# yzhang511/multi_modal_foundation_model

Measured on AMD Instinct MI355X. Metric: pretrain samples/sec (T=100 bins/modality, d_model=256, 5+5 layers, spike+behaviour masked pretraining step), higher is better.
Workload: dtype bf16; 1 GPU; BASELINE.json configs[1]: 1 session, ap(668 neurons)+behaviour(2), d_model=256, heads=8, mlp=512, 5 enc + 5 dec layers, T=100 (L=200 tokens), dropout 0.4/0.2, AdamW+OneCycleLR, mixed objectives; per_gpu_batch=1024, global_batch=1024, seq_len=200, parallelism=dp1

## Files before the change

### include/mmfm.h

```cpp
#ifndef MMFM_H
#define MMFM_H
#include <stdint.h>
#ifdef __cplusplus
extern "C" {
#endif

#define MMFM_VERSION 401
#define MMFM_F32 0
#define MMFM_BF16 1
#define MMFM_NULL_BIAS 1
#define MMFM_EMBED_OPTS 1
#define MMFM_MLP_DX_ONLY 1
#define MMFM_MLP_GELU 0
#define MMFM_MLP_RELU 1
#define MMFM_MLP_SIGMOID 2
#define MMFM_MLP_GELU_TANH 3

typedef void* mmfm_stream;

typedef struct {
    const void* state;
    uint32_t site;
    float p;
} mmfm_dropout;
// ... 253 lines not shown
int mmfm_optim_ranges_table(const mmfm_optim_range* ranges, int n_ranges, int64_t n, int hyper_rows, void* table_host, int64_t table_bytes);
int64_t mmfm_optim_ranges_workspace(int64_t n_chunks, int n_ranges);
int mmfm_grad_sumsq_ranges(const float* g, int64_t n, const mmfm_optim_range* ranges, int n_ranges, const void* table, int64_t n_chunks,
                           float coef_in, float max_norm, int skip_nonfinite, void* workspace, int64_t workspace_bytes,
                           mmfm_stream stream);
int mmfm_adamw_step_ranges(float* p, const float* g, float* m, float* v, void* p_bf16, int64_t n, const mmfm_optim_range* ranges,
                           int n_ranges, const void* table, int64_t n_chunks, const float* hyper, int hyper_rows,
                           const mmfm_optim_record* record, int skip_nonfinite, mmfm_stream stream);

#define MMFM_GRAD_ACCUM 1
#define MMFM_GRAD_STASH 0
#define MMFM_GRAD_ADD 1
int mmfm_grad_accumulate(float* g, float* stash, int64_t n, int64_t start, int64_t end, int mode, mmfm_stream stream);

#define MMFM_SESSION_LINEAR 1
typedef struct {
    int dtype;
    int B, T, P, N_max, S;
    int ld_pad;
    int ld_p;
    const int32_t* sid;
    const int32_t* n;
    const int64_t* w_off;
    const int64_t* b_off;
    const void* w; int64_t w_elems;
    const float* bias; int64_t b_elems;
} mmfm_session_desc;
int mmfm_session_reduce(const mmfm_session_desc* d, const void* x_pad, void* y, mmfm_stream stream);
int mmfm_session_expand(const mmfm_session_desc* d, const void* f, void* y_pad, mmfm_stream stream);
int mmfm_session_dw_chunks(int B, int S, int chunk);
int64_t mmfm_session_runs_ints(int B, int S, int chunk);
int64_t mmfm_session_dw_workspace(int B, int P, int N_max, int S, int chunk);
int mmfm_session_dw(const mmfm_session_desc* d, const void* a_pad, const void* q, const int32_t* runs, int chunk, float* dw, float* db,
                    int bias_from_pad, void* workspace, int64_t workspace_bytes, mmfm_stream stream);

#define MMFM_SPAN_PACK 1
#define MMFM_SPAN_CHUNK 4096
#define MMFM_SPAN_MAX 65536
int mmfm_span_gather(const float* G, float* stage, const int64_t* table, int n_spans, mmfm_stream stream);
int mmfm_span_scatter(const float* stage, float* G, const int64_t* table, int n_spans, mmfm_stream stream);

int mmfm_r2_series(const float* gt, const int64_t* gt_strides, const float* pred, const int64_t* pred_strides,
                   int G, int S, int C, float* out, mmfm_stream stream);
int64_t mmfm_bits_per_spike_workspace(int64_t R, int N);
int mmfm_bits_per_spike(const float* rates, const float* spikes, int64_t R, int N, float* out,
                        void* workspace, int64_t workspace_bytes, mmfm_stream stream);
int64_t mmfm_bits_per_spike_neurons_workspace(int64_t R, int N);
int mmfm_bits_per_spike_neurons(const float* rates, const float* spikes, int64_t R, int N, float* out,
                                void* workspace, int64_t workspace_bytes, mmfm_stream stream);


typedef struct {
    const float* W;
    const float* gamma;
    const float* beta;
    const float* bias;
    void* Wp;
    void* WpT;
    float* bp;
    int N, K;
    int tile0;
    int scalar_gain;
    void* WpP;
    void* WpTP;
} mmfm_prep_entry;
int mmfm_prep_weights(const mmfm_prep_entry* entries, int n_entries, int total_tiles, mmfm_stream stream);

typedef struct {
    int64_t R;
    int K, N;
    const void* x; int ldx;
    const void* w; int ldw;
    const float* bias;
    int ln; float eps;
    void* xhat; float* rstd;
    const void* residual; int ldr;
    void* y; int ldy;
    int stream_out;
    int rotate;
    int ln_bwd;
    const void* bwd_xhat; const float* bwd_rstd;
} mmfm_rowgemm_desc;
int mmfm_rowgemm(const mmfm_rowgemm_desc* d, mmfm_stream stream);

#define MMFM_ROWGEMM_MAX_GROUPS 8
typedef struct {
    int64_t R;
    int K, N;
    int groups;
    const void* x[MMFM_ROWGEMM_MAX_GROUPS]; int ldx;
    const void* w[MMFM_ROWGEMM_MAX_GROUPS]; int ldw;
    const float* bias[MMFM_ROWGEMM_MAX_GROUPS];
    void* y[MMFM_ROWGEMM_MAX_GROUPS]; int ldy;
    int ln; float eps;
    void* xhat; float* rstd;
    const void* residual; int ldr;
    int stream_out, rotate;
    int ln_bwd;
    const void* bwd_xhat; const float* bwd_rstd;
} mmfm_rowgemm_groups_desc;
int mmfm_rowgemm_groups(const mmfm_rowgemm_groups_desc* d, mmfm_stream stream);

typedef struct {
    int64_t R;
    const void* x; int ldx;
    float eps;
    const void* w_up; const float* b_up;
    const void* w_down; const float* b_down;
    mmfm_dropout drop;
    void* y; int ldy;
    void* xhat; float* rstd;
    const void* dy; int lddy;
    const void* w_down_t;
    const void* w_up_t;
    void* t1; void* g; void* du;
    void* dx; int lddx;
    int rotate;
    int scalenorm;
    int act;
    float act_beta;
} mmfm_mlp_desc;
int mmfm_mlp_fwd(const mmfm_mlp_desc* d, mmfm_stream stream);
int mmfm_mlp_bwd(const mmfm_mlp_desc* d, mmfm_stream stream);

int64_t mmfm_ln_linear_grad_workspace(int K);
int mmfm_ln_linear_grad(const float* Gdb, const float* W, const float* gamma, const float* beta, int N, int K,
                        float* dW, float* dbias, float* dgamma, float* dbeta, int accumulate_ln,
                        void* workspace, int64_t workspace_bytes, mmfm_stream stream);
int mmfm_sn_linear_grad(const float* Gdb, const float* W, const float* g, int N, int K, float* dW, float* dbias, float* dg,
                        int accumulate, void* workspace, int64_t workspace_bytes, mmfm_stream stream);

int mmfm_mt19937_jump(uint32_t* state624, int32_t* consumed, uint64_t n);
int mmfm_mt19937_jump_reset(void);

#define MMFM_MT_DEVICE 1
#define MMFM_MT_MAX_STREAMS 1024
#define MMFM_MT_TABLES 64
int mmfm_mt_plan(uint64_t n, int streams, int32_t* out_streams, int64_t* out_blocks);
int64_t mmfm_mt_workspace(uint64_t n, int streams);
int mmfm_mt_uniform(const uint32_t* state624, int32_t consumed, uint64_t skip, uint64_t n, float* out, int streams,
                    void* workspace, int64_t workspace_bytes, mmfm_stream stream);
int mmfm_mt_bernoulli(const uint32_t* state624, int32_t consumed, uint64_t skip, uint64_t n, float p, uint8_t* out, int streams,
                      void* workspace, int64_t workspace_bytes, mmfm_stream stream);
int mmfm_mt_corrupt(const uint32_t* state624, int32_t consumed, int B, int T, int N, const float* src, const uint8_t* cm,
                    int64_t sb, int64_t st, int64_t sn, float zero_ratio, float random_ratio, float* dst, int streams,
                    void* workspace, int64_t workspace_bytes, mmfm_stream stream);

#ifdef __cplusplus
}
#endif
#endif
```

### multi_modal_foundation_model_amd/_lib.py

```python
from __future__ import annotations

import ctypes as C
import os
import re

import torch

_HERE = os.path.dirname(os.path.abspath(__file__))
LIB_PATH = os.environ.get("MMFM_LIB") or os.path.join(_HERE, "libmmfm_hip.so")
HEADER_PATH = os.path.join(os.path.dirname(_HERE), "include", "mmfm.h")

F32, BF16 = 0, 1
ATTN_DIAG, ATTN_CAUSAL, ATTN_SEP = 1, 2, 4
ATTN_FAMILY_KEEPBIT_DH32, ATTN_FAMILY_KEEPBIT_LONG, ATTN_FAMILY_BF16, ATTN_FAMILY_BF16_TILED, ATTN_FAMILY_F32, ATTN_FAMILY_F32_TILED = range(1, 7)
ATTN_FAMILY_MASK, ATTN_FAMILY_BWD_SINGLE = 0xf, 0x10
ATTN_KEEPBIT_FAMILIES = (ATTN_FAMILY_KEEPBIT_DH32, ATTN_FAMILY_KEEPBIT_LONG)
GEMM_FAMILY_F32, GEMM_FAMILY_TILE128, GEMM_FAMILY_BIG256, GEMM_FAMILY_DW128, GEMM_FAMILY_DW256 = range(1, 6)
ACT_NONE, ACT_GELU, ACT_SOFTSIGN, ACT_GELU_GRAD, ACT_SOFTSIGN_GRAD, ACT_SOFTSIGN_GRAD_OUT = 0, 1, 2, 3, 4, 5
ACT_RELU, ACT_RELU_GRAD, ACT_SIGMOID, ACT_SIGMOID_GRAD, ACT_GELU_TANH, ACT_GELU_TANH_GRAD = 6, 7, 8, 9, 10, 11
(ACT_EMB_IDENTITY, ACT_EMB_IDENTITY_GRAD, ACT_EMB_RELU, ACT_EMB_RELU_GRAD, ACT_EMB_GELU, ACT_EMB_GELU_GRAD, ACT_EMB_SILU, ACT_EMB_SILU_GRAD,
 ACT_EMB_QUICK_GELU, ACT_EMB_QUICK_GELU_GRAD, ACT_EMB_GELU_TANH, ACT_EMB_GELU_TANH_GRAD, ACT_EMB_TANH, ACT_EMB_TANH_GRAD) = range(12, 26)
MLP_GELU, MLP_RELU, MLP_SIGMOID, MLP_GELU_TANH = 0, 1, 2, 3
LOSS_POISSON_LOG, LOSS_MSE, LOSS_POISSON_RATE, LOSS_L1, LOSS_SMOOTH_L1, LOSS_HUBER, LOSS_BCE_LOGITS = range(7)
LOSS_FULL = 1
# ... 119 lines not shown
    "mmfm_last_error": (C.c_char_p, []),
    "mmfm_device_check": (C.c_int, [_i]),
    "mmfm_rng_seed": (C.c_int, [_vp, C.c_uint64, _vp]),
    "mmfm_rng_advance": (C.c_int, [_vp, _vp]),
    "mmfm_gemm": (C.c_int, [C.POINTER(GemmDesc), _vp]),
    "mmfm_gemm_pair": (C.c_int, [_vp, _vp, _vp]),
    "mmfm_gemm_live": (C.c_int, [C.POINTER(GemmDesc), C.POINTER(LiveRows), _vp]),
    "mmfm_gemm_family": (C.c_int, [C.POINTER(GemmDesc), C.POINTER(LiveRows)]),
    "mmfm_gemm_pair_fused": (C.c_int, [C.POINTER(GemmDesc), C.POINTER(GemmDesc)]),
    "mmfm_live_bins": (C.c_int, [_vp, _i, _i, _vp, _vp]),
    "mmfm_gather_live_rows": (C.c_int, [_vp, _vp, _i, _i, _i64, _vp, _vp]),
    "mmfm_gemm_dw_tiles": (C.c_int, [_i, _i, _i]),
    "mmfm_reduce_slabs": (C.c_int, [_vp, _vp, _i64, _i, _i64, _i, _vp]),
    "mmfm_reduce_slabs_multi": (C.c_int, [_vp, _i, _i, _vp]),
    "mmfm_colsum_workspace": (C.c_int64, [_i64, _i]),
    "mmfm_colsum": (C.c_int, [_i, _vp, _i64, _i, _i, _vp, _i, _vp, _i64, _vp]),
    "mmfm_layernorm_fwd": (C.c_int, [_i, _vp, _vp, _vp, _vp, _vp, _vp, _i64, _i, _f, _i, _i, _vp]),
    "mmfm_layernorm_bwd_workspace": (C.c_int64, [_i64, _i]),
    "mmfm_layernorm_bwd": (C.c_int, [_i, _vp, _vp, _vp, _vp, _vp, _vp, _vp, _vp, _vp, _i, _i64, _i, _i, _i, _vp, _i64, _vp]),
    "mmfm_scalenorm_fwd": (C.c_int, [_i, _vp, _vp, _vp, _vp, _i64, _i, _f, _vp]),
    "mmfm_scalenorm_bwd_workspace": (C.c_int64, [_i64, _i]),
    "mmfm_scalenorm_bwd": (C.c_int, [_i, _vp, _vp, _vp, _vp, _vp, _vp, _vp, _i, _i64, _i, _vp, _i64, _vp]),
    "mmfm_attn_fwd": (C.c_int, [C.POINTER(AttnDesc), _vp]),
    "mmfm_attn_bwd": (C.c_int, [C.POINTER(AttnDesc), _vp]),
    "mmfm_attn_keepbits_bytes": (C.c_int64, [_i, _i, _i, _i]),
    "mmfm_attn_keep_prob": (C.c_float, [_f]),
    "mmfm_attn_family": (C.c_int, [C.POINTER(AttnDesc), _i]),
    "mmfm_attn_win_fwd": (C.c_int, [C.POINTER(AttnDesc), C.POINTER(AttnWindow), _vp]),
    "mmfm_attn_win_bwd": (C.c_int, [C.POINTER(AttnDesc), C.POINTER(AttnWindow), _vp]),
    "mmfm_attn_win_family": (C.c_int, [C.POINTER(AttnDesc), C.POINTER(AttnWindow), _i]),
    "mmfm_attn_pos_prep": (C.c_int, [_i, _i, C.POINTER(C.c_int32), C.POINTER(_vp), _vp, _vp]),
    "mmfm_mask_prep": (C.c_int, [_i, _i, _i, C.POINTER(_vp), C.POINTER(_i64), _vp, C.POINTER(_i64), _vp, _vp, _vp, _vp, _vp, _vp]),
    "mmfm_collate_csr": (C.c_int, [_i, _i, _i, _f, _vp, _vp, _vp, _vp, _vp, _vp, _vp, _vp, _vp, _vp, _vp]),
    "mmfm_stitch_fwd": (C.c_int, [_i, _vp, _vp, _vp, _vp, _vp, _vp, _vp, _i, _i, _i, _i, _i, _i, _vp]),
    "mmfm_stitch_fwd_live": (C.c_int, [_i, _vp, _vp, _vp, _vp, _vp, _vp, _vp, _vp, _i, _i, _i, _i, _i, _i, _vp]),
    "mmfm_stitch_bwd_live": (C.c_int, [_i, _vp, _vp, _vp, _vp, _vp, Dropout, _vp, _vp, _vp, _i, _i, _i, _i, _i, _i, _i, _i, _vp, _i64, _vp]),
    "mmfm_stitch_bwd_workspace": (C.c_int64, [_i, _i, _i, _i, _i, _i]),
    "mmfm_stitch_bwd": (C.c_int, [_i, _vp, _vp, _vp, _vp, Dropout, _vp, _vp, _vp, _i, _i, _i, _i, _i, _i, _i, _i, _vp, _i64, _vp]),
    "mmfm_mask_prep_seg": (C.c_int, [_i, _i, C.POINTER(C.c_int32), C.POINTER(_vp), C.POINTER(_i64), C.POINTER(_vp), C.POINTER(_i64), _vp, _vp, _vp, _vp,
                                     _vp, _vp]),
    "mmfm_stitch_fwd_seg": (C.c_int, [_i, _vp, _vp, _vp, _vp, _vp, _vp, _vp, _i, _i, _i, _i, _i, _i, _vp]),
    "mmfm_stitch_bwd_seg_workspace": (C.c_int64, [_i, _i, _i, _i, _i, _i, _i]),
    "mmfm_stitch_bwd_seg": (C.c_int, [_i, _vp, _vp, _vp, _vp, Dropout, _vp, _vp, _vp, _i, _i, _i, _i, _i, _i, _i, _i, _vp, _i64, _vp]),
    "mmfm_layernorm_fwd_seg": (C.c_int, [_i, _vp, _vp, _vp, _vp, _vp, _vp, _i64, _i, _f, _i, C.POINTER(C.c_int32), _vp]),
    "mmfm_layernorm_bwd_seg": (C.c_int, [_i, _vp, _vp, _vp, _vp, _vp, _vp, _vp, _vp, _vp, _i, _i64, _i, _i, C.POINTER(C.c_int32), _vp, _i64, _vp]),
    "mmfm_masked_loss_workspace": (C.c_int64, [_i64, _i]),
    "mmfm_masked_loss_fwd": (C.c_int, [_i, _i, _vp, _vp, _vp, _i, _i, _i64, _i, _vp, _vp, _i64, _vp]),
    "mmfm_masked_loss_kind_fwd": (C.c_int, [_i, _i, _f, _i, _vp, _vp, _vp, _i, _i, _i64, _i, _vp, _vp, _i64, _vp]),
    "mmfm_loss_finalize": (C.c_int, [_vp, _vp, _i, _vp, _vp, _vp]),
    "mmfm_masked_loss_bwd": (C.c_int, [_i, _i, _vp, _vp, _vp, _i, _i, _i64, _i, _vp, _vp, _vp, _vp]),
    "mmfm_masked_loss_kind_bwd": (C.c_int, [_i, _i, _f, _i, _vp, _vp, _vp, _i, _i, _i64, _i, _vp, _vp, _vp, _vp]),
    "mmfm_masked_loss_elem_workspace": (C.c_int64, [_i64, _i]),
    "mmfm_masked_loss_elem_fwd": (C.c_int, [_i, _i, _f, _i, _vp, _vp, _vp, _i64, _i64, _i64, _i, _i, _i, _vp, _vp, _vp, _i64, _vp]),
    "mmfm_masked_loss_elem_bwd": (C.c_int, [_i, _i, _f, _i, _vp, _vp, _vp, _i64, _i64, _i64, _i, _i, _i, _vp, _vp, _vp, _vp]),
    "mmfm_stage_masked": (C.c_int, [_i, _vp, _vp, _i64, _i64, _i64, _i, _i, _i, _vp, _i, _vp]),
    "mmfm_masked_loss_chan_workspace": (C.c_int64, [_i64, _i]),
    "mmfm_masked_loss_chan_fwd": (C.c_int, [_i, _i, _f, _i, _vp, _vp, _vp, _i, _i, _i64, _i, _vp, _i, _vp, _vp, _vp, _i64, _vp]),
    "mmfm_masked_loss_chan_bwd": (C.c_int, [_i, _i, _f, _i, _vp, _vp, _vp, _i, _i, _i64, _i, _vp, _i, _vp, _vp, _vp, _vp]),
    "mmfm_softmax_ce_workspace": (C.c_int64, [_i64, _i]),
    "mmfm_softmax_ce_fwd": (C.c_int, [_i, _vp, _vp, _vp, _f, _vp, _i, _i, _i64, _i, _vp, _vp, _vp, _i64, _vp]),
    "mmfm_softmax_ce_bwd": (C.c_int, [_i, _vp, _vp, _vp, _f, _vp, _i, _i, _i64, _i, _vp, _vp, _vp, _vp, _vp]),
    "mmfm_argmax_confusion": (C.c_int, [_i, _vp, _vp, _vp, _i, _i, _i64, _i, _vp, _vp]),
    "mmfm_dropout_apply": (C.c_int, [_i, _vp, _vp, _i64, _i, Dropout, _vp]),
    "mmfm_cast_f32_to_bf16": (C.c_int, [_vp, _vp, _i64, _vp]),
    "mmfm_adamw_step": (C.c_int, [_vp, _vp, _vp, _vp, _vp, _i64, _vp, _vp]),
    "mmfm_optim_ranges_chunks": (C.c_int64, [C.POINTER(OptimRange), _i, _i64, _i]),
    "mmfm_optim_ranges_table_bytes": (C.c_int64, [_i64, _i]),
    "mmfm_optim_ranges_table": (C.c_int, [C.POINTER(OptimRange), _i, _i64, _i, _vp, _i64]),
    "mmfm_optim_ranges_workspace": (C.c_int64, [_i64, _i]),
    "mmfm_grad_sumsq_ranges": (C.c_int, [_vp, _i64, C.POINTER(OptimRange), _i, _vp, _i64, _f, _f, _i, _vp, _i64, _vp]),
    "mmfm_adamw_step_ranges": (C.c_int, [_vp, _vp, _vp, _vp, _vp, _i64, C.POINTER(OptimRange), _i, _vp, _i64, _vp, _i, _vp, _i, _vp]),
    "mmfm_grad_accumulate": (C.c_int, [_vp, _vp, _i64, _i64, _i64, _i, _vp]),
    "mmfm_session_reduce": (C.c_int, [C.POINTER(SessionDesc), _vp, _vp, _vp]),
    "mmfm_session_expand": (C.c_int, [C.POINTER(SessionDesc), _vp, _vp, _vp]),
    "mmfm_session_dw_chunks": (C.c_int, [_i, _i, _i]),
    "mmfm_session_runs_ints": (C.c_int64, [_i, _i, _i]),
    "mmfm_session_dw_workspace": (C.c_int64, [_i, _i, _i, _i, _i]),
    "mmfm_session_dw": (C.c_int, [C.POINTER(SessionDesc), _vp, _vp, _vp, _i, _vp, _vp, _i, _vp, _i64, _vp]),
    "mmfm_span_gather": (C.c_int, [_vp, _vp, _vp, _i, _vp]),
    "mmfm_span_scatter": (C.c_int, [_vp, _vp, _vp, _i, _vp]),
    "mmfm_prep_weights": (C.c_int, [_vp, _i, _i, _vp]),
    "mmfm_rowgemm": (C.c_int, [C.POINTER(RowGemmDesc), _vp]),
    "mmfm_rowgemm_groups": (C.c_int, [C.POINTER(RowGemmGroupsDesc), _vp]),
    "mmfm_mlp_fwd": (C.c_int, [C.POINTER(MlpDesc), _vp]),
    "mmfm_mlp_bwd": (C.c_int, [C.POINTER(MlpDesc), _vp]),
    "mmfm_ln_linear_grad_workspace": (C.c_int64, [_i]),
    "mmfm_ln_linear_grad": (C.c_int, [_vp, _vp, _vp, _vp, _i, _i, _vp, _vp, _vp, _vp, _i, _vp, _i64, _vp]),
    "mmfm_sn_linear_grad": (C.c_int, [_vp, _vp, _vp, _i, _i, _vp, _vp, _vp, _i, _vp, _i64, _vp]),
    "mmfm_r2_series": (C.c_int, [_vp, C.POINTER(_i64), _vp, C.POINTER(_i64), _i, _i, _i, _vp, _vp]),
    "mmfm_bits_per_spike_workspace": (C.c_int64, [_i64, _i]),
    "mmfm_bits_per_spike": (C.c_int, [_vp, _vp, _i64, _i, _vp, _vp, _i64, _vp]),
    "mmfm_bits_per_spike_neurons_workspace": (C.c_int64, [_i64, _i]),
    "mmfm_bits_per_spike_neurons": (C.c_int, [_vp, _vp, _i64, _i, _vp, _vp, _i64, _vp]),
    "mmfm_mt19937_jump": (C.c_int, [_vp, C.POINTER(C.c_int32), C.c_uint64]),
    "mmfm_mt19937_jump_reset": (C.c_int, []),
    "mmfm_mt_plan": (C.c_int, [C.c_uint64, _i, C.POINTER(C.c_int32), C.POINTER(_i64)]),
    "mmfm_mt_workspace": (C.c_int64, [C.c_uint64, _i]),
    "mmfm_mt_uniform": (C.c_int, [_vp, C.c_int32, C.c_uint64, C.c_uint64, _vp, _i, _vp, _i64, _vp]),
    "mmfm_mt_bernoulli": (C.c_int, [_vp, C.c_int32, C.c_uint64, C.c_uint64, _f, _vp, _i, _vp, _i64, _vp]),
    "mmfm_mt_corrupt": (C.c_int, [_vp, C.c_int32, _i, _i, _i, _vp, _vp, _i64, _i64, _i64, _f, _f, _vp, _i, _vp, _i64, _vp]),
}

_lib = None


def header_symbols():
    with open(HEADER_PATH) as f:
        src = f.read()
    src = re.sub(r"/\*.*?\*/", "", src, flags=re.S)
    return sorted(set(re.findall(r"\b(mmfm_[a-z0-9_]+)\s*\(", src)))


def lib():
    global _lib
    if _lib is None:
        if not os.path.exists(LIB_PATH):
            raise ImportError(f"{LIB_PATH} is missing: the HIP extension is not built and there is no CPU "
                              "fallback.  Run `python -c 'import __graft_entry__ as g; g.build()'`.")
        l = C.CDLL(LIB_PATH)
        for name, (res, args) in _PROTOS.items():
            fn = getattr(l, name)
            fn.restype, fn.argtypes = res, args
        _lib = l
    return _lib


def check(rc, what=""):
    if rc != 0:
        raise MmfmError(f"{what} failed (code {rc}): {lib().mmfm_last_error().decode(errors='replace')}")
```

### multi_modal_foundation_model_amd/csrc/rowgemm.hip

```cpp
#define MMFM_ACT_LOAD_AUX 2
#include "rowchain.h"
#include <stdlib.h>
#include <algorithm>
#include <type_traits>

using namespace rowchain;

namespace {

constexpr int NT = 256, NW = 4;

constexpr int BIAS_MAX = 1024;

template <int KP, int LN, bool NTS, int NWV>
__global__ __launch_bounds__(NWV * 64, (KP == 1 ? 2 : 1)) void rowgemm_kernel(const mmfm_rowgemm_desc d) {
    constexpr int NT = NWV * 64, NW = NWV;
    __shared__ __attribute__((aligned(16))) char smem[LDS_BYTES + NW * STG_BYTES + BIAS_MAX * 4];
    const int t = threadIdx.x, lane = t & 63, wave = __builtin_amdgcn_readfirstlane(t >> 6), m = lane & 31, h = lane >> 5;
    const int npair = d.N >> 6, cpp = 2 * npair * KP;
    const int64_t npass = (d.R + 32 * NW - 1) / (32 * NW);
    const int my_passes = blockIdx.x < npass ? (int)((npass - 1 - blockIdx.x) / gridDim.x) + 1 : 0;
    if (my_passes == 0) return;
    const uint16_t* W = reinterpret_cast<const uint16_t*>(d.w);
    const int ldw = d.ldw;
// ... 537 lines not shown
    opnd x[16];
    load_rows_lines<4>(stg, x, gbuf(d.x[0], xbytes), row_of(0), ldxb, lane, m, h);
    for (int pi = 0; pi < my_passes; ++pi) {
        const uint32_t wrow0 = row_of(pi);
        const uint32_t nrow0 = pi + 1 < my_passes ? row_of(pi + 1) : (uint32_t)(npass * 32 * NW);
        {
            Lines xl[4];
#pragma unroll
            for (int tp = 0; tp < 4; ++tp) xl[tp] = fetch_lines(XH, wrow0, 512u, 128u * tp, lane);
#pragma unroll
            for (int tp = 0; tp < 4; ++tp) stage_lines(xstash + tp * STG_BYTES, xl[tp], lane);
        }
        float rs = ld4f(RS, (wrow0 + m) * 4u);
        f32x16 acc[8];
#pragma unroll
        for (int tt = 0; tt < 8; ++tt) acc[tt] = zero16();
        for (int q = 0; q < npiece; ++q) {
            const int nq = q + 1 < npiece ? q + 1 : 0;
            const uint32_t nrow = q + 1 < npiece ? wrow0 : nrow0;
            const GBuf XN = gbuf(pick8(d.x, KP == 1 ? nq : nq >> 1), xbytes);
            const uint32_t ncol = KP == 1 ? 0u : 512u * (uint32_t)(nq & 1);
            Lines L[4];
#pragma unroll
            for (int s = 0; s < 4; ++s) L[s] = fetch_lines(XN, nrow, ldxb, ncol + 128u * s, lane);
            opnd xn[16];
#pragma unroll
            for (int tt = 0; tt < 8; ++tt) {
                if (tt == 2) {
#pragma unroll
                    for (int s = 0; s < 4; ++s) {
                        stage_lines(stg, L[s], lane);
#pragma unroll
                        for (int s4 = 0; s4 < 4; ++s4) xn[4 * s + s4] = unstage_opnd(stg, s4, m, h);
                    }
                }
                uint32_t slot;
                if (tt < 2) { RINGA_SYNC(src, slot, 16); acc[tt] = mma16a<4>(slot, fr, x, acc[tt], [&](int g_) { RINGA_PIECE(g_); }); }
                else { RINGA_SYNC(src, slot, 0); acc[tt] = mma16a<4>(slot, fr, x, acc[tt], [&](int g_) { RINGA_PIECE(g_); }); }
            }
#pragma unroll
            for (int s = 0; s < 16; ++s) x[s] = xn[s];
        }
        float s1 = 0.f, s2 = 0.f;
#pragma unroll
        for (int tp = 0; tp < 4; ++tp) {
#pragma unroll
            for (int j = 0; j < 2; ++j) {
                const f32x16 xt = unstage_tile(xstash + tp * STG_BYTES, j, m, h);
#pragma unroll
                for (int i = 0; i < 16; ++i) { s1 += acc[2 * tp + j][i]; s2 = fmaf(acc[2 * tp + j][i], xt[i], s2); }
            }
        }
        s1 = xhalf(s1);
        s2 = xhalf(s2);
        norm_bwd_stats<NORM>(s1, s2, rs);
        Lines rl4[4];
#pragma unroll
        for (int tp = 0; tp < 4; ++tp) rl4[tp] = fetch_lines(RES, wrow0, ldrb, 128u * tp, lane);
#pragma unroll
        for (int tp = 0; tp < 4; ++tp) {
            const Lines& rl = rl4[tp];
            f32x16 o[2];
#pragma unroll
            for (int j = 0; j < 2; ++j) {
                const f32x16 xt = unstage_tile(xstash + tp * STG_BYTES, j, m, h);
#pragma unroll
                for (int i = 0; i < 16; ++i) o[j][i] = rs * (acc[2 * tp + j][i] - s1 - xt[i] * s2);
            }
            stage_lines(stg, rl, lane);
#pragma unroll
            for (int j = 0; j < 2; ++j) {
                const f32x16 r = unstage_tile(stg, j, m, h);
#pragma unroll
                for (int i = 0; i < 16; ++i) o[j][i] += r[i];
            }
            stage_tile(stg, 0, m, h, o[0]);
            stage_tile(stg, 1, m, h, o[1]);
            flush_lines<false>(stg, Y, wrow0, ldyb, 128u * tp, lane);
        }
    }
}
#pragma clang diagnostic pop

__global__ __launch_bounds__(256) void prep_weights_kernel(const mmfm_prep_entry* __restrict__ E, int ne) {
    __shared__ float tile[32][33];
    int e = 0;
    while (e + 1 < ne && (int)blockIdx.x >= E[e + 1].tile0) ++e;
    const mmfm_prep_entry en = E[e];
    const int n0 = ((int)blockIdx.x - en.tile0) * 32;
    const int tx = threadIdx.x & 31, ty = threadIdx.x >> 5;
    uint16_t* Wp = reinterpret_cast<uint16_t*>(en.Wp);
    uint16_t* WpT = reinterpret_cast<uint16_t*>(en.WpT);
    uint16_t* WpP = reinterpret_cast<uint16_t*>(en.WpP);
    uint16_t* WpTP = reinterpret_cast<uint16_t*>(en.WpTP);
    auto perm = [](int i) { return (i & ~12) | ((i & 4) << 1) | ((i & 8) >> 1); };
    float dot[4] = {0.f, 0.f, 0.f, 0.f};
    const float gs = en.scalar_gain ? en.gamma[0] : 1.f;
    for (int k0 = 0; k0 < en.K; k0 += 32) {
        const int k = k0 + tx;
        const float g = en.scalar_gain ? gs : (en.gamma && k < en.K) ? en.gamma[k] : 1.f;
        const float bt = (en.beta && k < en.K && !en.scalar_gain) ? en.beta[k] : 0.f;
#pragma unroll
        for (int j = 0; j < 4; ++j) {
            const int n = n0 + ty + 8 * j;
            const float v = (n < en.N && k < en.K) ? en.W[(size_t)n * en.K + k] : 0.f;
            const float w = v * g;
            dot[j] = fmaf(v, bt, dot[j]);
            if (Wp && n < en.N && k < en.K) Wp[(size_t)n * en.K + k] = f2bf(w);
            if (WpP && n < en.N && k < en.K && perm(k) < en.K) WpP[(size_t)n * en.K + perm(k)] = f2bf(w);
            tile[ty + 8 * j][tx] = w;
        }
        __syncthreads();
        if (WpT || WpTP) {
#pragma unroll
            for (int j = 0; j < 4; ++j) {
                const int kk = k0 + ty + 8 * j, n = n0 + tx;
                if (kk < en.K && n < en.N) {
                    if (WpT) WpT[(size_t)kk * en.N + n] = f2bf(tile[tx][ty + 8 * j]);
                    if (WpTP && perm(n) < en.N) WpTP[(size_t)kk * en.N + perm(n)] = f2bf(tile[tx][ty + 8 * j]);
                }
            }
        }
        __syncthreads();
    }
    if (en.bp) {
#pragma unroll
        for (int j = 0; j < 4; ++j) {
            float r = dot[j];
#pragma unroll
            for (int o = 16; o > 0; o >>= 1) r += __shfl_xor(r, o);
            const int n = n0 + ty + 8 * j;
            if (tx == 0 && n < en.N) en.bp[n] = (en.bias ? en.bias[n] : 0.f) + r;
        }
    }
}

int grid_for(int64_t R, int per_cu, int nw = NW) {
    const int64_t npass = (R + 32 * nw - 1) / (32 * nw);
    return (int)std::max<int64_t>(1, std::min<int64_t>(npass, 256 * per_cu));
}

}

extern "C" int mmfm_rowgemm(const mmfm_rowgemm_desc* dp, mmfm_stream stream) {
    const mmfm_rowgemm_desc d = *dp;
    MMFM_REQUIRE(d.x && d.w && d.y && d.R > 0, "mmfm_rowgemm: null operand / empty problem");
    MMFM_REQUIRE(d.K == 256 || d.K == 512 || d.K == 768, "mmfm_rowgemm: K = %d (256, 512 or 768 only)", d.K);
    MMFM_REQUIRE(d.N > 0 && d.N % 64 == 0, "mmfm_rowgemm: N = %d must be a positive multiple of 64", d.N);
    MMFM_REQUIRE(d.ldx % 8 == 0 && d.ldw % 8 == 0 && d.ldy % 8 == 0 && d.ldx >= d.K && d.ldw >= d.K && d.ldy >= d.N,
                 "mmfm_rowgemm: leading dimensions (%d, %d, %d) must be multiples of 8 and cover the rows", d.ldx, d.ldw, d.ldy);
    auto al16 = [](const void* p) { return ((uintptr_t)p & 15) == 0; };
    MMFM_REQUIRE(al16(d.x) && al16(d.w) && al16(d.y) && al16(d.residual) && al16(d.xhat) && al16(d.bwd_xhat) && al16(d.bias),
                 "mmfm_rowgemm: operands must be 16-byte aligned");
    MMFM_REQUIRE(!d.residual || (d.ldr % 8 == 0 && d.ldr >= d.N), "mmfm_rowgemm: ldr %d", d.ldr);
    MMFM_REQUIRE(d.ln >= 0 && d.ln <= 2 && d.ln_bwd >= 0 && d.ln_bwd <= 2, "mmfm_rowgemm: ln = %d, ln_bwd = %d (0, 1 = LayerNorm, 2 = ScaleNorm)", d.ln, d.ln_bwd);
    MMFM_REQUIRE(!d.ln || d.K == 256, "mmfm_rowgemm: the norm prologue needs K = 256");
    const int64_t maxld = std::max<int64_t>(std::max(d.ldx, d.ldy), std::max(d.ldr, 256));
    MMFM_REQUIRE((d.R + 128) * maxld * 2 < (int64_t)1 << 31, "mmfm_rowgemm: tensors beyond 2 GiB are not addressable by the 32-bit buffer offsets");
    MMFM_REQUIRE(d.N <= BIAS_MAX, "mmfm_rowgemm: N = %d > %d", d.N, BIAS_MAX);
    static const int per_cu_env = [] { const char* e = getenv("MMFM_ROWGEMM_WG_PER_CU"); return e ? atoi(e) : 0; }();
    hipStream_t st = (hipStream_t)stream;
    if (d.ln_bwd) {
        MMFM_REQUIRE(d.N == 256 && d.bwd_xhat && d.bwd_rstd && !d.ln && !d.bias, "mmfm_rowgemm: ln_bwd needs N = 256, x_hat, rstd, no bias/ln");
        const bool sn = d.ln_bwd == 2;
        if (d.K == 256) {
            dim3 grid(grid_for(d.R, per_cu_env > 0 ? per_cu_env : 1, 4)), block(512);
            if (sn) hipLaunchKernelGGL((rowgemm_lnbwd8_kernel<1, 2>), grid, block, 0, st, d);
            else hipLaunchKernelGGL((rowgemm_lnbwd8_kernel<1, 1>), grid, block, 0, st, d);
        } else {
            dim3 grid(grid_for(d.R, per_cu_env > 0 ? per_cu_env : 1)), block(NT);
            static const int ring_env = [] { const char* e = getenv("MMFM_ROWGEMM_RING"); return (e ? atoi(e) : 3) & 2; }();
            constexpr int LDS_L = RINGA_SLOTS * CHUNK + NW * STG_BYTES + NW * 4 * STG_BYTES;
#define LNB_A(KP, NORM)                                                                                                     \
            {                                                                                                               \
                if (int rc = mmfm_lds_opt_in(reinterpret_cast<const void*>(rowgemm_lnbwd_a_kernel<KP, NORM>), LDS_L, "mmfm_rowgemm")) return rc; \
                hipLaunchKernelGGL((rowgemm_lnbwd_a_kernel<KP, NORM>), grid, block, LDS_L, st, d);                           \
            }
            if (ring_env && d.K == 512) { if (sn) LNB_A(2, 2) else LNB_A(2, 1) }
            else if (ring_env) { if (sn) LNB_A(3, 2) else LNB_A(3, 1) }
            else if (d.K == 512) { if (sn) hipLaunchKernelGGL((rowgemm_lnbwd_kernel<2, 2>), grid, block, 0, st, d); else hipLaunchKernelGGL((rowgemm_lnbwd_kernel<2, 1>), grid, block, 0, st, d); }
            else { if (sn) hipLaunchKernelGGL((rowgemm_lnbwd_kernel<3, 2>), grid, block, 0, st, d); else hipLaunchKernelGGL((rowgemm_lnbwd_kernel<3, 1>), grid, block, 0, st, d); }
#undef LNB_A
        }
    } else {
#define RG_LAUNCH(KP, LN)                                                                                   \
    if (d.stream_out) hipLaunchKernelGGL((rowgemm_kernel<KP, LN, true, 4>), grid, block, 0, st, d);         \
    else hipLaunchKernelGGL((rowgemm_kernel<KP, LN, false, 4>), grid, block, 0, st, d);
        if (d.K != 256) {
            dim3 grid(grid_for(d.R, per_cu_env > 0 ? per_cu_env : 1, 4)), block(256);
            if (d.K == 512) { RG_LAUNCH(2, 0) } else { RG_LAUNCH(3, 0) }
        } else {
            dim3 grid(grid_for(d.R, per_cu_env > 0 ? per_cu_env : 2, 4)), block(256);
            static const int ring_env = [] { const char* e = getenv("MMFM_ROWGEMM_RING"); return (e ? atoi(e) : 3) & 1; }();
            if (ring_env && (!d.residual || (d.N == 256 && !d.ln))) {
                constexpr int LDS_A = RINGA_SLOTS * CHUNK + 4 * STG_BYTES + BIAS_MAX * 4;
#define RGA_LAUNCH(LN, NTS, NPV)                                                                                            \
                {                                                                                                          \
                    if (int rc = mmfm_lds_opt_in(reinterpret_cast<const void*>(rowgemm_a_kernel<LN, NTS, NPV>), LDS_A, "mmfm_rowgemm")) return rc; \
                    hipLaunchKernelGGL((rowgemm_a_kernel<LN, NTS, NPV>), grid, block, LDS_A, st, d);                        \
                }
#define RGA_LAUNCH2(LN, NPV) if (d.stream_out) RGA_LAUNCH(LN, true, NPV) else RGA_LAUNCH(LN, false, NPV)
                const int64_t npass = (d.R + 127) / 128;
                const int np_all = d.N >> 6;
                static const int nsplit_env = [] { const char* e = getenv("MMFM_ROWGEMM_NSPLIT"); return e ? atoi(e) : 1; }();
                const int ny = (nsplit_env && npass < 128) ? (int)std::max<int64_t>(1, std::min<int64_t>(np_all, 512 / npass)) : 1;
                if (d.residual) {
                    if (ny >= 4) { grid.y = 4; RGA_LAUNCH2(0, 1) } else { RGA_LAUNCH2(0, 4) }
                } else {
                    grid.y = (unsigned)((np_all + (np_all + ny - 1) / ny - 1) / ((np_all + ny - 1) / ny));
                    if (d.ln == 2) RGA_LAUNCH2(2, 0)
                    else if (d.ln) RGA_LAUNCH2(1, 0)
                    else RGA_LAUNCH2(0, 0)
                }
#undef RGA_LAUNCH2
#undef RGA_LAUNCH
            } else if (d.ln == 2) { RG_LAUNCH(1, 2) } else if (d.ln) { RG_LAUNCH(1, 1) } else { RG_LAUNCH(1, 0) }
        }
#undef RG_LAUNCH
    }
    MMFM_LAUNCH_CHECK("mmfm_rowgemm");
    return 0;
}

extern "C" int mmfm_rowgemm_groups(const mmfm_rowgemm_groups_desc* dp, mmfm_stream stream) {
    const mmfm_rowgemm_groups_desc d = *dp;
    MMFM_REQUIRE(d.groups >= 1 && d.groups <= GROUPS_MAX && d.R > 0, "mmfm_rowgemm_groups: groups = %d (1 .. %d), R = %lld", d.groups, GROUPS_MAX, (long long)d.R);
    MMFM_REQUIRE(d.ln >= 0 && d.ln <= 2 && d.ln_bwd >= 0 && d.ln_bwd <= 2 && (d.ln != 0) != (d.ln_bwd != 0),
                 "mmfm_rowgemm_groups: ln = %d, ln_bwd = %d: exactly one of them must be 1 (LayerNorm) or 2 (ScaleNorm)", d.ln, d.ln_bwd);
    MMFM_REQUIRE(d.ldx % 8 == 0 && d.ldw % 8 == 0 && d.ldy % 8 == 0 && d.ldx >= d.K && d.ldw >= d.K && d.ldy >= d.N,
                 "mmfm_rowgemm_groups: leading dimensions (%d, %d, %d) must be multiples of 8 and cover the rows", d.ldx, d.ldw, d.ldy);
    auto al16 = [](const void* p) { return ((uintptr_t)p & 15) == 0; };
    const int nx = d.ln_bwd ? d.groups : 1, ny = d.ln_bwd ? 1 : d.groups;
    uintptr_t wmin = (uintptr_t)d.w[0];
    for (int g = 0; g < d.groups; ++g) {
        MMFM_REQUIRE(d.w[g] && al16(d.w[g]) && al16(d.bias[g]), "mmfm_rowgemm_groups: group %d: weights NULL or operands not 16-byte aligned", g);
        MMFM_REQUIRE(g >= nx || (d.x[g] && al16(d.x[g])), "mmfm_rowgemm_groups: group %d: x NULL or not 16-byte aligned", g);
        MMFM_REQUIRE(g >= ny || (d.y[g] && al16(d.y[g])), "mmfm_rowgemm_groups: group %d: y NULL or not 16-byte aligned", g);
        wmin = std::min(wmin, (uintptr_t)d.w[g]);
    }
    MMFM_REQUIRE(al16(d.residual) && al16(d.xhat) && al16(d.bwd_xhat), "mmfm_rowgemm_groups: operands must be 16-byte aligned");
    GroupOff wo = {};
    const int64_t wbytes = (int64_t)(d.ln_bwd ? 256 : d.N) * d.ldw * 2;
    for (int g = 0; g < d.groups; ++g) {
        const int64_t off = (int64_t)((uintptr_t)d.w[g] - wmin);
        MMFM_REQUIRE(off + wbytes < (int64_t)1 << 31, "mmfm_rowgemm_groups: group %d: weights more than 2 GiB from the first group's", g);
        wo.w[g] = (uint32_t)off;
    }
    const int64_t maxld = std::max<int64_t>(std::max(d.ldx, d.ldy), std::max(d.ldr, 256));
    MMFM_REQUIRE((d.R + 256) * maxld * 2 < (int64_t)1 << 31, "mmfm_rowgemm_groups: tensors beyond 2 GiB are not addressable by the 32-bit buffer offsets");
    static const int per_cu_env = [] { const char* e = getenv("MMFM_ROWGEMM_WG_PER_CU"); return e ? atoi(e) : 0; }();
    hipStream_t st = (hipStream_t)stream;
    const void* wbase = (const void*)wmin;
    if (d.ln_bwd) {
        MMFM_REQUIRE(d.N == 256 && (d.K == 256 || d.K == 512) && d.bwd_xhat && d.bwd_rstd,
                     "mmfm_rowgemm_groups: ln_bwd needs N = 256, K = 256 or 512 (got %d, %d), x_hat and rstd", d.N, d.K);
        MMFM_REQUIRE(!d.residual || (d.ldr % 8 == 0 && d.ldr >= d.N), "mmfm_rowgemm_groups: ldr %d", d.ldr);
        dim3 grid(grid_for(d.R, per_cu_env > 0 ? per_cu_env : 1)), block(NT);
        constexpr int LDS_L = RINGA_SLOTS * CHUNK + NW * STG_BYTES + NW * 4 * STG_BYTES;
#define GLNB(KP, NORM)                                                                                                      \
        {                                                                                                                   \
            if (int rc = mmfm_lds_opt_in(reinterpret_cast<const void*>(rowgemm_groups_lnbwd_kernel<KP, NORM>), LDS_L, "mmfm_rowgemm_groups")) return rc; \
            hipLaunchKernelGGL((rowgemm_groups_lnbwd_kernel<KP, NORM>), grid, block, LDS_L, st, d, wbase, wo);              \
        }
        if (d.K == 256) { if (d.ln_bwd == 2) GLNB(1, 2) else GLNB(1, 1) }
        else { if (d.ln_bwd == 2) GLNB(2, 2) else GLNB(2, 1) }
#undef GLNB
    } else {
        MMFM_REQUIRE(d.K == 256, "mmfm_rowgemm_groups: the norm prologue needs K = 256 (got %d)", d.K);
        MMFM_REQUIRE(d.N >= 64 && d.N <= 1024 && (d.N & (d.N - 1)) == 0, "mmfm_rowgemm_groups: N = %d must be 64, 128, 256, 512 or 1024", d.N);
        MMFM_REQUIRE(d.groups * d.N <= GBIAS_MAX, "mmfm_rowgemm_groups: groups * N = %d > %d", d.groups * d.N, GBIAS_MAX);
        MMFM_REQUIRE(!d.residual, "mmfm_rowgemm_groups: the grouped forward takes no residual");
        int nps = 0;
        while ((64 << nps) < d.N) ++nps;
        dim3 grid(grid_for(d.R, per_cu_env > 0 ? per_cu_env : 2, 4)), block(256);
        constexpr int LDS_A = RINGA_SLOTS * CHUNK + 4 * STG_BYTES + GBIAS_MAX * 4;
        const int64_t npass = (d.R + 127) / 128;
        const int np_all = (d.N >> 6) * d.groups;
        static const int nsplit_env = [] { const char* e = getenv("MMFM_ROWGEMM_NSPLIT"); return e ? atoi(e) : 1; }();
        const int nyb = (nsplit_env && npass < 128) ? (int)std::max<int64_t>(1, std::min<int64_t>(np_all, 512 / npass)) : 1;
        grid.y = (unsigned)((np_all + (np_all + nyb - 1) / nyb - 1) / ((np_all + nyb - 1) / nyb));
#define GFWD(LN, NTS)                                                                                                       \
        {                                                                                                                   \
            if (int rc = mmfm_lds_opt_in(reinterpret_cast<const void*>(rowgemm_groups_a_kernel<LN, NTS>), LDS_A, "mmfm_rowgemm_groups")) return rc; \
            hipLaunchKernelGGL((rowgemm_groups_a_kernel<LN, NTS>), grid, block, LDS_A, st, d, wbase, wo, nps);              \
        }
        if (d.ln == 2) { if (d.stream_out) GFWD(2, true) else GFWD(2, false) }
        else { if (d.stream_out) GFWD(1, true) else GFWD(1, false) }
#undef GFWD
    }
    MMFM_LAUNCH_CHECK("mmfm_rowgemm_groups");
    return 0;
}

extern "C" int mmfm_prep_weights(const mmfm_prep_entry* entries_dev, int n_entries, int total_tiles, mmfm_stream stream) {
    MMFM_REQUIRE(entries_dev && n_entries > 0 && total_tiles > 0, "mmfm_prep_weights: empty table");
    hipLaunchKernelGGL(prep_weights_kernel, dim3(total_tiles), dim3(256), 0, (hipStream_t)stream, entries_dev, n_entries);
    MMFM_LAUNCH_CHECK("mmfm_prep_weights");
    return 0;
}
```

Measured before the change: 37580 samples/s.

## Add two-workgroup-per-CU LN-backward rowgemm kernel with async x prefetch

Adds a new LayerNorm-backward row GEMM kernel that keeps the A-operand in registers, fetched asynchronously one block ahead, instead of staging it through extra LDS. This cuts LDS use so two workgroups fit per CU. It is used for K=512/768 (and grouped K=512) when the row count exceeds 256 passes and the weight ring is enabled. The aim is better latency hiding through higher occupancy, at the risk of register pressure under the 2-wave launch bound. A query function is exported so callers can see which form will run.

```diff
diff --git a/include/mmfm.h b/include/mmfm.h
--- a/include/mmfm.h
+++ b/include/mmfm.h
@@ -359,6 +359,7 @@
     const void* bwd_xhat; const float* bwd_rstd;
 } mmfm_rowgemm_desc;
 int mmfm_rowgemm(const mmfm_rowgemm_desc* d, mmfm_stream stream);
+int mmfm_rowgemm_lnbwd_form(int64_t R, int K);
 
 #define MMFM_ROWGEMM_MAX_GROUPS 8
 typedef struct {
diff --git a/multi_modal_foundation_model_amd/_lib.py b/multi_modal_foundation_model_amd/_lib.py
--- a/multi_modal_foundation_model_amd/_lib.py
+++ b/multi_modal_foundation_model_amd/_lib.py
@@ -225,6 +225,7 @@
     "mmfm_prep_weights": (C.c_int, [_vp, _i, _i, _vp]),
     "mmfm_rowgemm": (C.c_int, [C.POINTER(RowGemmDesc), _vp]),
     "mmfm_rowgemm_groups": (C.c_int, [C.POINTER(RowGemmGroupsDesc), _vp]),
+    "mmfm_rowgemm_lnbwd_form": (C.c_int, [_i64, _i]),
     "mmfm_mlp_fwd": (C.c_int, [C.POINTER(MlpDesc), _vp]),
     "mmfm_mlp_bwd": (C.c_int, [C.POINTER(MlpDesc), _vp]),
     "mmfm_ln_linear_grad_workspace": (C.c_int64, [_i]),
diff --git a/multi_modal_foundation_model_amd/csrc/rowgemm.hip b/multi_modal_foundation_model_amd/csrc/rowgemm.hip
--- a/multi_modal_foundation_model_amd/csrc/rowgemm.hip
+++ b/multi_modal_foundation_model_amd/csrc/rowgemm.hip
@@ -643,6 +643,138 @@
 }
 #pragma clang diagnostic pop
 
+#pragma clang diagnostic push
+#pragma clang diagnostic ignored "-Winline-asm"
+__device__ __forceinline__ void fetch_lines_async(Lines& L, const GBuf& b, uint32_t wrow0, uint32_t ldb, uint32_t colb, int lane) {
+#pragma unroll
+    for (int i = 0; i < 4; ++i) {
+        const uint32_t off = (wrow0 + 8 * i + (lane >> 3)) * ldb + colb + 16 * (lane & 7);
+        asm volatile("buffer_load_dwordx4 %0, %1, %2, 0 offen nt" : "=v"(L.v[i]) : "v"(off), "s"(b.rs) : "memory");
+    }
+}
+template <int NORM>
+__global__ __launch_bounds__(256, 2) void rowgemm_lnbwd2_kernel(const mmfm_rowgemm_groups_desc d, const void* wbase, const GroupOff wo) {
+    constexpr int NT = 256, NW = 4, RING_B = RINGA_SLOTS * CHUNK;
+    extern __shared__ __attribute__((aligned(16))) char smem[];
+    const int t = threadIdx.x, lane = t & 63, wave = __builtin_amdgcn_readfirstlane(t >> 6), m = lane & 31, h = lane >> 5;
+    const int kb = d.K >> 6, kc = 2 * kb, nblk = d.groups * kb;
+    const int64_t npass = (d.R + 32 * NW - 1) / (32 * NW);
+    const int my_passes = blockIdx.x < npass ? (int)((npass - 1 - blockIdx.x) / gridDim.x) + 1 : 0;
+    if (my_passes == 0) return;
+    const __amdgpu_buffer_rsrc_t rs_w = wbuf(wbase);
+    const uint32_t ldwb = (uint32_t)d.ldw * 2u;
+    int src_g = 0, src_c = 0;
+    auto src = [&](int) {
+        AChunk c;
+        c.rs = rs_w; c.off = __builtin_amdgcn_readfirstlane(pick8(wo.w, src_g) + 64u * (uint32_t)src_c); c.ldb = ldwb; c.kind = 2;
+        if (++src_c == kc) { src_c = 0; if (++src_g == d.groups) src_g = 0; }
+        return c;
+    };
+    char* stg = smem + RING_B + wave * STG_BYTES;
+    const GBuf Y = gbuf(d.y[0], d.R * d.ldy * 2), RES = gbuf(d.residual, d.R * d.ldr * 2);
+    const GBuf XH = gbuf(d.bwd_xhat, d.R * 512), RS = gbuf(d.bwd_rstd, d.R * 4);
+    const uint32_t ldxb = d.ldx * 2, ldyb = d.ldy * 2, ldrb = d.ldr * 2;
+    const int64_t xbytes = d.R * d.ldx * 2;
+    auto row_of = [&](int pi) { return (uint32_t)(((int64_t)(blockIdx.x + (int64_t)pi * gridDim.x) * NW + wave) * 32); };
+    int xs_g = 0, xs_c = 0, xs_pi = 0;
+    auto xfetch = [&](Lines& L) {
+        const uint32_t row0 = xs_pi < my_passes ? row_of(xs_pi) : (uint32_t)(npass * 32 * NW);
+        fetch_lines_async(L, gbuf(pick8(d.x, xs_g), xbytes), row0, ldxb, 128u * (uint32_t)xs_c, lane);
+        if (++xs_c == kb) { xs_c = 0; if (++xs_g == d.groups) { xs_g = 0; ++xs_pi; } }
+    };
+    const ALane<NT> ring_al = alane_init<NT>(t, 0u, ldwb);
+    const AFrag fr = afrag_init(m, h);
+    RINGA_DECL(NT);
+    Lines L0;
+    xfetch(L0);
+    RINGA_START((uint32_t)(uintptr_t)(__attribute__((address_space(3))) char*)smem, my_passes * nblk * 2, src);
+    f32x16 acc[8];
+#define L2_READS(SET, Q) do { ALDS_READ_B(wv[SET][0], slot, fr, 2 * (Q), 0); ALDS_READ_B(wv[SET][1], slot, fr, 2 * (Q), 1);          \
+                              ALDS_READ_B(wv[SET][2], slot, fr, 2 * (Q) + 1, 0); ALDS_READ_B(wv[SET][3], slot, fr, 2 * (Q) + 1, 1); } while (0)
+#define L2_MMAS(SET, Q, X0, X1) do { acc[2 * (Q)] = mfma_u4(wv[SET][0], X0, acc[2 * (Q)]); acc[2 * (Q) + 1] = mfma_u4(wv[SET][2], X0, acc[2 * (Q) + 1]); \
+                                     acc[2 * (Q)] = mfma_u4(wv[SET][1], X1, acc[2 * (Q)]); acc[2 * (Q) + 1] = mfma_u4(wv[SET][3], X1, acc[2 * (Q) + 1]); \
+                                     __builtin_amdgcn_sched_barrier(0); } while (0)
+#define L2_STEP(X0, X1, EXTRA)                                                                           \
+        {                                                                                                \
+            uint32_t slot;                                                                               \
+            RINGA_SYNC(src, slot, EXTRA);                                                                \
+            uint4 wv[2][4];                                                                              \
+            L2_READS(0, 0); L2_READS(1, 1);                                                              \
+            ALDS_WAITN(4); L2_MMAS(0, 0, X0, X1); RINGA_PIECE(0); L2_READS(0, 2);                        \
+            ALDS_WAITN(4); L2_MMAS(1, 1, X0, X1); RINGA_PIECE(1); L2_READS(1, 3);                        \
+            ALDS_WAITN(4); L2_MMAS(0, 2, X0, X1); RINGA_PIECE(2);                                        \
+            ALDS_WAITN(0); L2_MMAS(1, 3, X0, X1); RINGA_PIECE(3);                                        \
+        }
+#define L2_BLOCK(L, FETCH)                                                                               \
+        {                                                                                                \
+            vm_wait_n<8>();                                                                              \
+            stage_lines(stg, L, lane);                                                                   \
+            opnd xa[2];                               \
+            xa[0] = unstage_opnd(stg, 0, m, h); xa[1] = unstage_opnd(stg, 1, m, h);                      \
+            if (FETCH) xfetch(L);                                                                        \
+            L2_STEP(xa[0], xa[1], (FETCH) ? 4 : 0)                                                       \
+            xa[0] = unstage_opnd(stg, 2, m, h); xa[1] = unstage_opnd(stg, 3, m, h);                      \
+            L2_STEP(xa[0], xa[1], (FETCH) ? 4 : 0)                                                       \
+        }
+    for (int pi = 0; pi < my_passes; ++pi) {
+        const uint32_t wrow0 = row_of(pi);
+#pragma unroll
+        for (int tt = 0; tt < 8; ++tt) acc[tt] = zero16();
+        for (int b = 1; b < nblk; ++b) L2_BLOCK(L0, 1)
+        L2_BLOCK(L0, 0)
+        int le = lane;
+        asm volatile("" : "+v"(le));
+        const int me = le & 31, he = le >> 5;
+        Lines la = fetch_lines(XH, wrow0, 512u, 0u, le), lb = fetch_lines(XH, wrow0, 512u, 128u, le);
+        float rs = 0.f, s1 = 0.f, s2 = 0.f;
+#pragma unroll
+        for (int tp = 0; tp < 4; ++tp) {
+            Lines& lx = (tp & 1) ? lb : la;
+            stage_lines(stg, lx, le);
+            if (tp < 2) lx = fetch_lines(XH, wrow0, 512u, 128u * (tp + 2), le);
+            else if (tp == 2) lx = fetch_lines(XH, wrow0, 512u, 0u, le);
+            else { lx = fetch_lines(RES, wrow0, ldrb, 0u, le); rs = ld4f(RS, (wrow0 + me) * 4u); }
+#pragma unroll
+            for (int j = 0; j < 2; ++j) {
+                const f32x16 xt = unstage_tile(stg, j, me, he);
+#pragma unroll
+                for (int i = 0; i < 16; ++i) { s1 += acc[2 * tp + j][i]; s2 = fmaf(acc[2 * tp + j][i], xt[i], s2); }
+            }
+        }
+        s1 = xhalf(s1);
+        s2 = xhalf(s2);
+        norm_bwd_stats<NORM>(s1, s2, rs);
+#pragma unroll
+        for (int tp = 0; tp < 4; ++tp) {
+            f32x16 o[2];
+            stage_lines(stg, la, le);
+            if (tp + 1 < 4) la = fetch_lines(XH, wrow0, 512u, 128u * (tp + 1), le);
+#pragma unroll
+            for (int j = 0; j < 2; ++j) {
+                const f32x16 xt = unstage_tile(stg, j, me, he);
+#pragma unroll
+                for (int i = 0; i < 16; ++i) o[j][i] = rs * (acc[2 * tp + j][i] - s1 - xt[i] * s2);
+            }
+            stage_lines(stg, lb, le);
+            if (tp + 1 < 4) lb = fetch_lines(RES, wrow0, ldrb, 128u * (tp + 1), le);
+#pragma unroll
+            for (int j = 0; j < 2; ++j) {
+                const f32x16 r = unstage_tile(stg, j, me, he);
+#pragma unroll
+                for (int i = 0; i < 16; ++i) o[j][i] += r[i];
+                stage_tile(stg, j, me, he, o[j]);
+            }
+            flush_lines<false>(stg, Y, wrow0, ldyb, 128u * tp, le);
+            if (tp == 1) xfetch(L0);
+        }
+    }
+#undef L2_BLOCK
+#undef L2_STEP
+#undef L2_MMAS
+#undef L2_READS
+}
+#pragma clang diagnostic pop
+
 __global__ __launch_bounds__(256) void prep_weights_kernel(const mmfm_prep_entry* __restrict__ E, int ne) {
     __shared__ float tile[32][33];
     int e = 0;
@@ -699,6 +831,27 @@
 int grid_for(int64_t R, int per_cu, int nw = NW) {
     const int64_t npass = (R + 32 * nw - 1) / (32 * nw);
     return (int)std::max<int64_t>(1, std::min<int64_t>(npass, 256 * per_cu));
+}
+
+int lnbwd_wg_per_cu(int64_t R) {
+    static const int ring_env = [] { const char* e = getenv("MMFM_ROWGEMM_RING"); return (e ? atoi(e) : 3) & 2; }();
+    const char* e = getenv("MMFM_ROWGEMM_LNBWD_WG");
+    const int v = e ? atoi(e) : 0;
+    if (v == 1 || v == 2) return v;
+    if (!ring_env) return 1;
+    return (R + 32 * NW - 1) / (32 * NW) > 256 ? 2 : 1;
+}
+constexpr int LDS_L2 = RINGA_SLOTS * CHUNK + NW * STG_BYTES;
+int launch_lnbwd2(const mmfm_rowgemm_groups_desc& g, int norm, const void* wbase, const GroupOff& wo, hipStream_t st, const char* who) {
+    dim3 grid(grid_for(g.R, 2)), block(NT);
+    if (norm == 2) {
+        if (int rc = mmfm_lds_opt_in(reinterpret_cast<const void*>(rowgemm_lnbwd2_kernel<2>), LDS_L2, who)) return rc;
+        hipLaunchKernelGGL((rowgemm_lnbwd2_kernel<2>), grid, block, LDS_L2, st, g, wbase, wo);
+    } else {
+        if (int rc = mmfm_lds_opt_in(reinterpret_cast<const void*>(rowgemm_lnbwd2_kernel<1>), LDS_L2, who)) return rc;
+        hipLaunchKernelGGL((rowgemm_lnbwd2_kernel<1>), grid, block, LDS_L2, st, g, wbase, wo);
+    }
+    return 0;
 }
 
 }
@@ -728,6 +881,12 @@
             dim3 grid(grid_for(d.R, per_cu_env > 0 ? per_cu_env : 1, 4)), block(512);
             if (sn) hipLaunchKernelGGL((rowgemm_lnbwd8_kernel<1, 2>), grid, block, 0, st, d);
             else hipLaunchKernelGGL((rowgemm_lnbwd8_kernel<1, 1>), grid, block, 0, st, d);
+        } else if (lnbwd_wg_per_cu(d.R) == 2) {
+            mmfm_rowgemm_groups_desc g = {};
+            g.R = d.R; g.K = d.K; g.N = d.N; g.groups = 1;
+            g.x[0] = d.x; g.ldx = d.ldx; g.w[0] = d.w; g.ldw = d.ldw; g.y[0] = d.y; g.ldy = d.ldy;
+            g.residual = d.residual; g.ldr = d.ldr; g.ln_bwd = d.ln_bwd; g.bwd_xhat = d.bwd_xhat; g.bwd_rstd = d.bwd_rstd;
+            if (int rc = launch_lnbwd2(g, d.ln_bwd, d.w, GroupOff{}, st, "mmfm_rowgemm")) return rc;
         } else {
             dim3 grid(grid_for(d.R, per_cu_env > 0 ? per_cu_env : 1)), block(NT);
             static const int ring_env = [] { const char* e = getenv("MMFM_ROWGEMM_RING"); return (e ? atoi(e) : 3) & 2; }();
@@ -783,6 +942,8 @@
     return 0;
 }
 
+extern "C" int mmfm_rowgemm_lnbwd_form(int64_t R, int K) { return K == 512 || K == 768 ? lnbwd_wg_per_cu(R) : 1; }
+
 extern "C" int mmfm_rowgemm_groups(const mmfm_rowgemm_groups_desc* dp, mmfm_stream stream) {
     const mmfm_rowgemm_groups_desc d = *dp;
     MMFM_REQUIRE(d.groups >= 1 && d.groups <= GROUPS_MAX && d.R > 0, "mmfm_rowgemm_groups: groups = %d (1 .. %d), R = %lld", d.groups, GROUPS_MAX, (long long)d.R);
@@ -816,6 +977,11 @@
         MMFM_REQUIRE(d.N == 256 && (d.K == 256 || d.K == 512) && d.bwd_xhat && d.bwd_rstd,
                      "mmfm_rowgemm_groups: ln_bwd needs N = 256, K = 256 or 512 (got %d, %d), x_hat and rstd", d.N, d.K);
         MMFM_REQUIRE(!d.residual || (d.ldr % 8 == 0 && d.ldr >= d.N), "mmfm_rowgemm_groups: ldr %d", d.ldr);
+        if (d.K == 512 && lnbwd_wg_per_cu(d.R) == 2) {
+            if (int rc = launch_lnbwd2(d, d.ln_bwd, wbase, wo, st, "mmfm_rowgemm_groups")) return rc;
+            MMFM_LAUNCH_CHECK("mmfm_rowgemm_groups");
+            return 0;
+        }
         dim3 grid(grid_for(d.R, per_cu_env > 0 ? per_cu_env : 1)), block(NT);
         constexpr int LDS_L = RINGA_SLOTS * CHUNK + NW * STG_BYTES + NW * 4 * STG_BYTES;
 #define GLNB(KP, NORM)                                                                                                      \
```

New measurement: 38140 samples/s (median of 6 runs). 1.01x the previous value.
